# worldlife123/cbench_BaSIC

Hardware: AMD Instinct MI355X
Metric: encode+decode Mpix/s (higher is better)
Workload: dtype f32; 1 GPU; hyperprior codec N=128 M=192 (lossy_graph_scalable_exp_hp), synthetic 3x256x256 images (image i = manual_seed(i), rand), 256 images per GPU per step resident in HBM, compress+decompress incl. bitstream D2H/H2D, 6 concurrent stream workers per GPU (step k on worker k mod W: whole batches, W in flight); images_per_gpu=256, workers=6, rans_waves_per_workgroup=8, batches_in_flight=6, parallelism=image-sharded x1, RCCL all-reduce of metric sums

## Files before the change

cbench_basic_amd/_lib.py:

```python
import ctypes
import os

_HERE = os.path.dirname(os.path.abspath(__file__))
LIB_PATH = os.path.join(_HERE, "libbasic_hip.so")

OK, ERR_INVALID, ERR_NOT_INIT, ERR_HIP, ERR_OVERFLOW, ERR_NO_DEVICE = 0, -1, -2, -3, -4, -5
IMAGE_CHW, IMAGE_HWC = 0, 1
PIXEL_U8, PIXEL_F32 = 0, 1


class BasicHipError(RuntimeError):
    pass


class BasicHipInvalid(BasicHipError, ValueError):
    """A call the library refuses (BASIC_ERR_INVALID / BASIC_ERR_NOT_INIT): a ValueError, as the reference's pybind11 layer
    raises, and like every other failure of the library a BasicHipError."""


_lib = None

c_i32p = ctypes.c_void_p
_I, _L, _P, _F = ctypes.c_int, ctypes.c_int64, ctypes.c_void_p, ctypes.c_float

# ... 41 lines not shown
    "basic_rate_refine_dev": (_I, [_P, _I, _I, _P, _I, _P, _P, _P]),
    "basic_hp_session_set_rate_targets": (_I, [_P, _P, _I, _P, _I, _I]),
    "basic_hp_session_rate_result": (_I, [_P, _P, _P, _P, _I]),
    "basic_eb_quantize_index_dev": (_I, [_P, _P, _I, _I, _I, _P, _P, _P, _P]),
    "basic_eb_dequantize_dev": (_I, [_P, _P, _I, _I, _I, _P, _P]),
    "basic_i32_to_f32_dev": (_I, [_P, _L, _P, _P]),
    "basic_pgm_gauss_encode_group_dev": (_I, [_P, _P, _I, _I, _I, _P, _L, _P, _I, _P, _P, _L, _L, _P, _P]),
    "basic_pgm_gauss_index_group_dev": (_I, [_P, _I, _I, _I, _P, _L, _P, _I, _P, _L, _L, _P]),
    "basic_pgm_gauss_scatter_group_dev": (_I, [_P, _P, _I, _I, _I, _P, _L, _L, _L, _P, _P]),
    "basic_gauss_nll_per_image_dev": (_I, [_P, _P, _I, _I, _I, _I, _F, _F, _P, _P]),
    "basic_gauss_nll_per_image_q_dev": (_I, [_P, _P, _I, _I, _I, _P, _I, _F, _F, _P, _P]),
    "basic_eb_nll_per_image_dev": (_I, [_P, _P, _I, _I, _I, _F, _P, _P]),
    "basic_conv_plan_create": (_I, [_P, _P, _I, _I, _I, _I, _I, _I, _I, _I, _P, _P, _I, _I, _P]),
    "basic_conv_plan_out_hw": (_I, [_P, _I, _I, _P, _P]),
    "basic_conv_forward_dev": (_I, [_P, _P, _I, _I, _I, _P, _P]),
    "basic_conv_plan_channels": (_I, [_P, _P, _P]),
    "basic_hp_session_create": (_I, [_P, _I, _P, _I, _P, _I, _P, _I, _P, _I, _P, _P, _I, _F, _P, _P]),
    "basic_hp_encode_bound": (_L, [_P, _I, _I, _I]),
    "basic_hp_encode_images": (_I, [_P, _P, _I, _I, _I, _I, _P, _L, _P, _P]),
    "basic_hp_encode_result": (_I, [_P, _P, _L, _P]),
    "basic_hp_decoded_shape": (_I, [_P, _P, _L, _P, _P, _P, _P]),
    "basic_hp_decode_images": (_I, [_P, _P, _L, _P, _L, _P]),
    "basic_image_u8_to_f32_dev": (_I, [_P, _I, _I, _I, _I, _I, _P, _P]),
    "basic_image_f32_to_u8_dev": (_I, [_P, _I, _I, _I, _I, _I, _P, _P]),
    "basic_image_sse_u8_dev": (_I, [_P, _I, _P, _I, _I, _I, _I, _I, _P, _P]),
    "basic_image_tiles_u8_to_f32_dev": (_I, [_P, _I, _I, _I, _I, _I, _I, _I, _I, _I, _I, _I, _I, _P, _P]),
    "basic_image_tiles_f32_to_u8_dev": (_I, [_P, _I, _I, _I, _I, _I, _I, _I, _I, _I, _I, _I, _P, _I, _I, _I, _P]),
    "basic_image_tiles_overlap_u8_to_f32_dev": (_I, [_P, _I, _I, _I, _I, _I, _I, _I, _I, _I, _I, _I, _I, _P, _P]),
    "basic_image_tiles_blend_dev": (_I, [_P, _I, _I, _I, _I, _I, _I, _I, _I, _I, _I, _I, _P, _I, _I, _P]),
    "basic_image_tiles_last_path": (_I, [_P]),
# ... 102 lines not shown
```

cbench_basic_amd/csrc/conv.hip:

```cpp
#include "common.h"

#include <algorithm>
#include <cmath>
#include <cstdlib>
#include <cstring>
#include <new>
#include <vector>

using namespace basic;

namespace {
thread_local bool g_dynamic_tiles = false;
}
namespace basic {
bool set_dynamic_tiles(bool on)
{
    const bool prev = g_dynamic_tiles;
    g_dynamic_tiles = on;
    return prev;
}
}

namespace {

// ... 15 lines not shown
constexpr int kPSlotsFused = 6;
constexpr int kFusedCK = 4;
constexpr int kMaxCoutPerLaunch = 192;
constexpr int kSplitBelowBlocks = 384;
constexpr int kPackTail = 32 * 32 * 8 + 2048;

struct TapLaunch {
    const float *in;
    float *out;
    const float *wpack;
    const float *wrow;
    const float *bias;
    int64_t split_wstride;
    const float *gammaT;
    const float *beta;
    int batch, cin, cin_pad, cout, coutp;
    int out_ctotal, co_base;
    int in_h, in_w, out_h, out_w;
    int mh, mw;
    int s_in, s_out, oy0, ox0;
    int ntaps, dymin, dxmin;
    int tb_log, th_log, tw_log;
    int ph, pw, pwp;
    int patch4;
    int act;
    int tiles_y, tiles_x;
    signed char dy[kMaxTaps], dx[kMaxTaps];
};

__device__ __forceinline__ int xcd_tile(int b, int n)
// ... 655 lines not shown
        }
    };
    if (gdn) {
        __syncthreads();
        const f32x4 *src = reinterpret_cast<const f32x4 *>(g.gammaT);
        f32x4 *dst = reinterpret_cast<f32x4 *>(gl);
#pragma unroll
        for (int sl = 0; sl < 128 * 32 * 4 / 4 / kSplitThreads; ++sl) dst[sl * kSplitThreads + tid_e] = src[sl * kSplitThreads + tid_e];
        __syncthreads();
    }
    finish(acc);
    finish(acc2);

    const Pos ep = pos_of(tid_e);
    const int my = ep.my, mx = ep.mx, be = b0 + ep.tb;
    if (my < g.mh && mx < g.mw && be < g.batch) {
        const int oy = my * g.s_out + g.oy0, ox = mx * g.s_out + g.ox0;
        const int64_t oplane = static_cast<int64_t>(g.out_h) * g.out_w;
        float *o = g.out + (static_cast<int64_t>(be) * g.out_ctotal + g.co_base) * oplane + static_cast<int64_t>(oy) * g.out_w + ox;
#pragma unroll
        for (int m = 0; m < MT; ++m)
#pragma unroll
            for (int r = 0; r < 16; ++r) {
                const int co = 32 * m + 8 * (r >> 2) + 4 * khalf_e + (r & 3);
                if (co < g.cout) {
                    f32x2 v2;
                    v2[0] = apply_act(acc[m][r], g.act);
                    v2[1] = apply_act(acc2[m][r], g.act);
                    *reinterpret_cast<f32x2 *>(o + co * oplane) = v2;
                }
            }
    }
}

template <int KH, bool PATCH>
hipError_t launch_split(const TapLaunch &g, const u32x4 *ws, const int *kw, const unsigned *amax, int blocks, hipStream_t st)
{
    const hipError_t e = ensure_max_lds(reinterpret_cast<const void *>(conv_split_f16_kernel<KH, 3, 2, PATCH>));
    if (e != hipSuccess) return e;
    hipLaunchKernelGGL((conv_split_f16_kernel<KH, 3, 2, PATCH>), dim3(blocks), dim3(kSplitThreads),
                       PATCH ? kSplitLdsPatchBytes : kSplitLdsBytes, st, g, ws, kw, amax);
    return hipGetLastError();
}

constexpr int kFirstSlots = 10;

// ... 975 lines not shown
    BASIC_HIP_TRY(hipGetLastError());
    return BASIC_OK;
}
}

extern "C" int basic_conv_plan_launches(const basic_conv_plan *p, int batch, int in_h, int in_w)
{
    int oh = 0, ow = 0;
    if (!p || batch < 1 || basic_conv_plan_out_hw(p, in_h, in_w, &oh, &ow)) return -1;
    if (p->d_wsm) return 1;
    int n = 0;
    for_each_launch(p, choose_launches(p, batch, oh, ow, nullptr), oh, ow, [&](const Chunk &, const Phase &, int, int) { ++n; return BASIC_OK; });
    return n;
}

extern "C" int basic_conv_forward_dev(const basic_conv_plan *p, const float *d_in, int batch, int in_h, int in_w,
                                      float *d_out, void *hip_stream)
{
    BASIC_REQUIRE(p && d_in && d_out && batch >= 1, "conv_forward: bad argument");
    int oh = 0, ow = 0;
    int rc = basic_conv_plan_out_hw(p, in_h, in_w, &oh, &ow);
    if (rc) return rc;
    if (p->d_wsm) return launch_small_deconv(p, d_in, batch, in_h, in_w, d_out, as_stream(hip_stream));
    const LaunchChoice choice = choose_launches(p, batch, oh, ow, d_out);
    bool amax_done = false;
    return for_each_launch(p, choice, oh, ow, [&](const Chunk &ch, const Phase &ph, int mh, int mw) -> int {
        TapLaunch g{};
        g.in = d_in; g.out = d_out; g.wpack = ph.d_wpack; g.wrow = ph.d_wrow; g.split_wstride = ph.split_wstride; g.bias = ch.d_bias; g.gammaT = p->d_gammaT; g.beta = p->d_beta;
        g.batch = batch; g.cin = p->cin; g.cin_pad = ph.ntaps ? ph.cin_pad : 0; g.cout = ch.cout; g.coutp = ch.coutp; g.out_ctotal = p->cout; g.co_base = ch.co0;
        g.in_h = in_h; g.in_w = in_w; g.out_h = oh; g.out_w = ow;
        g.s_in = p->s_in; g.s_out = p->s_out; g.oy0 = ph.oy0; g.ox0 = ph.ox0;
        g.mh = mh; g.mw = mw;
        g.ntaps = ph.ntaps; g.dymin = ph.dymin; g.dxmin = ph.dxmin;
        std::memcpy(g.dy, ph.dy, sizeof(g.dy));
        std::memcpy(g.dx, ph.dx, sizeof(g.dx));
        g.act = p->act;
        const int kCK = ph.ck;
        if (choice.split_f16 && ph.d_wsplit) {
            const TileShape ts = tile_shape(g.mh, g.mw, kSplitWaves * 32);
            const int tw = ts.tw, th = ts.th, tb = ts.tb;
            if (static_cast<int64_t>(tb) * p->cin * in_h * in_w * 4 < (1ll << 31)) {
// ... 1 lines not shown
                g.tiles_y = (g.mh + th - 1) / th;
                g.tiles_x = (g.mw + tw - 1) / tw;
                const int blocks = ((batch + tb - 1) / tb) * g.tiles_y * g.tiles_x;
                hipStream_t st = as_stream(hip_stream);
                const u32x4 *ws = static_cast<const u32x4 *>(ph.d_wsplit);
                BASIC_REQUIRE(ph.kw == 3 && ph.kwb == 2 && (ph.kh == 3 || ph.kh == 2), "conv_forward: split-fp16 plan / kernel instantiation mismatch");
                if (!amax_done) {
                    auto *pm = const_cast<basic_conv_plan *>(p);
                    if (pm->amax_cap < batch) {
                        if (pm->d_amax) BASIC_HIP_TRY(hipFree(pm->d_amax));
                        pm->d_amax = nullptr; pm->amax_cap = 0;
                        BASIC_HIP_TRY(hipMalloc(&pm->d_amax, sizeof(unsigned) * batch));
                        pm->amax_cap = batch;
                    }
                    BASIC_HIP_TRY(hipMemsetAsync(pm->d_amax, 0, sizeof(unsigned) * batch, st));
                    const int64_t n = static_cast<int64_t>(p->cin) * in_h * in_w;
                    const int per_img = static_cast<int>(std::min<int64_t>(64, std::max<int64_t>(1, n / 4096)));
                    hipLaunchKernelGGL(image_absmax_kernel, dim3(batch * per_img), dim3(256), 0, st, d_in, n, per_img, pm->d_amax);
                    BASIC_HIP_TRY(hipGetLastError());
                    amax_done = true;
                }
                const bool patch = choice.split_patch && g.s_in == 1 && tb * (th + ph.kh - 1) * (tw + ph.kw - 1) <= kSplitPatchPos;
                const unsigned *am = p->d_amax;
                const hipError_t e = ph.kh == 3 ? (patch ? launch_split<3, true>(g, ws, ph.d_wsplit_k, am, blocks, st) : launch_split<3, false>(g, ws, ph.d_wsplit_k, am, blocks, st))
                                                : (patch ? launch_split<2, true>(g, ws, ph.d_wsplit_k, am, blocks, st) : launch_split<2, false>(g, ws, ph.d_wsplit_k, am, blocks, st));
                BASIC_HIP_TRY(e);
                return BASIC_OK;
            }
        }
        const int threads = 64 * ph.waves, tile_pos = 32 * ph.waves;
        const TileShape ts = tile_shape(g.mh, g.mw, tile_pos);
        const int tw = ts.tw;
        int th = ts.th, tb = ts.tb;
        const bool first_layer_path = ch.mt == 4 && ch.nsplit == 1 && ph.waves == 8 && ph.kh == 5 && ph.kw == 5 &&
                                      ph.cin_pad == kCK && kCK == 4 && ch.cout == 128 && p->d_gammaT;
        g.ph = (th - 1) * g.s_in + ph.span_y;
        g.pw = (tw - 1) * g.s_in + ph.span_x;
        g.patch4 = (ph.waves == 8 && !first_layer_path && in_w % 4 == 0 && (reinterpret_cast<uintptr_t>(d_in) & 15) == 0) ? 1 : 0;
        g.pwp = g.patch4 ? (g.pw + 3 + 3) / 4 * 4 : (g.pw | 1);
        int punit = g.patch4 ? 4 : 1;
        const int mtp = mtile_pitch(ch.mt);
        const int wl_floats = g.ntaps * kCK * 32 * mtp, gam_floats = 32 * 32 * mtp;
        const int wl_pad = ((wl_floats > gam_floats ? wl_floats : gam_floats) + 4 * threads - 1) / (4 * threads) * (4 * threads);
        auto patch_slots_needed = [&](int tbv) { return (tbv * kCK * g.ph * g.pwp / punit + threads - 1) / threads; };
// ... 55 lines not shown
                default: set_error("conv_forward: fused phases need <= 4 accumulator tiles"); rc = BASIC_ERR_INVALID;
            }
            return rc;
        }
        switch (ch.mt) {
            case 1: rc = launch_mt<1>(g, ph.kh, ph.kw, ph.ck, ph.waves, blocks, ch.nsplit, lds_bytes, st); break;
            case 2: rc = launch_mt<2>(g, ph.kh, ph.kw, ph.ck, ph.waves, blocks, ch.nsplit, lds_bytes, st); break;
            case 3: rc = launch_mt<3>(g, ph.kh, ph.kw, ph.ck, ph.waves, blocks, ch.nsplit, lds_bytes, st); break;
            case 4: rc = launch_mt<4>(g, ph.kh, ph.kw, ph.ck, ph.waves, blocks, ch.nsplit, lds_bytes, st); break;
            case 5: rc = launch_mt<5>(g, ph.kh, ph.kw, ph.ck, ph.waves, blocks, ch.nsplit, lds_bytes, st); break;
            case 6: rc = launch_mt<6>(g, ph.kh, ph.kw, ph.ck, ph.waves, blocks, ch.nsplit, lds_bytes, st); break;
            default: set_error("conv_forward: cout > 192 unsupported"); rc = BASIC_ERR_INVALID;
        }
        return rc;
    });
}
```

cbench_basic_amd/csrc/entropy.hip:

```cpp
#include "ans_common.h"

using namespace basic;

namespace {

constexpr int kBlock = 256;

inline int grid_for(int64_t n)
{
    int64_t g = (n + kBlock - 1) / kBlock;
    if (g > 256 * 8) g = 256 * 8;
    if (g < 1) g = 1;
    return static_cast<int>(g);
}

__device__ __forceinline__ float round_even(float v) { return rintf(v); }

__global__ void gc_quantize_index_kernel(const float *__restrict__ y, const float *__restrict__ scales, int64_t n,
                                         const float *__restrict__ table, int table_len, float bound,
                                         int32_t *__restrict__ symbols, int32_t *__restrict__ indexes,
                                         float *__restrict__ yhat)
{
    extern __shared__ float s_table[];
    __shared__ int s_unsorted;
// ... 248 lines not shown
__global__ void eb_dequantize_kernel(const int32_t *__restrict__ symbols, const float *__restrict__ medians,
                                     int64_t total, int channels, int hw, float *__restrict__ zhat)
{
    for (int64_t i = static_cast<int64_t>(blockIdx.x) * blockDim.x + threadIdx.x; i < total;
         i += static_cast<int64_t>(gridDim.x) * blockDim.x) {
        const int c = static_cast<int>((i / hw) % channels);
        zhat[i] = static_cast<float>(symbols[i]) + medians[c];
    }
}

__global__ void i32_to_f32_kernel(const int32_t *__restrict__ in, int64_t n, float *__restrict__ out)
{
    for (int64_t i = static_cast<int64_t>(blockIdx.x) * blockDim.x + threadIdx.x; i < n;
         i += static_cast<int64_t>(gridDim.x) * blockDim.x)
        out[i] = static_cast<float>(in[i]);
}

__global__ void lanes_pack_kernel(const int32_t *__restrict__ sym, const int32_t *__restrict__ idx, int64_t total, int positions,
                                  int lanes, int width, int32_t *__restrict__ sym_out, int32_t *__restrict__ idx_out)
{
    for (int64_t i = static_cast<int64_t>(blockIdx.x) * blockDim.x + threadIdx.x; i < total;
         i += static_cast<int64_t>(gridDim.x) * blockDim.x) {
        const int64_t run = i / width;
        const int l = static_cast<int>(i - run * width);
        const int64_t bk = run / positions;
        const int p = static_cast<int>(run - bk * positions);
        const int64_t b = bk / lanes;
        const int k = static_cast<int>(bk - b * lanes);
        const int64_t src = ((b * positions + p) * lanes + k) * width + l;
        sym_out[i] = sym[src];
// ... 338 lines not shown
    hipLaunchKernelGGL(eb_dequantize_kernel, dim3(grid_for(total)), dim3(kBlock), 0, as_stream(hip_stream), d_symbols,
                       d_medians, total, channels, hw, d_zhat);
    BASIC_HIP_TRY(hipGetLastError());
    return BASIC_OK;
}

extern "C" int basic_i32_to_f32_dev(const int32_t *d_in, int64_t n, float *d_out, void *hip_stream)
{
    BASIC_REQUIRE(d_in && d_out && n >= 0, "i32_to_f32: bad argument");
    if (n == 0) return BASIC_OK;
    hipLaunchKernelGGL(i32_to_f32_kernel, dim3(grid_for(n)), dim3(kBlock), 0, as_stream(hip_stream), d_in, n, d_out);
    BASIC_HIP_TRY(hipGetLastError());
    return BASIC_OK;
}

extern "C" int basic_lanes_pack_dev(const int32_t *d_sym, const int32_t *d_idx, int batch, int positions, int channels, int lanes,
                                    int32_t *d_sym_out, int32_t *d_idx_out, void *hip_stream)
{
    BASIC_REQUIRE(d_sym && d_idx && d_sym_out && d_idx_out && batch >= 1 && positions >= 1 && channels >= 1 && lanes >= 1 &&
                      channels % lanes == 0 && d_sym_out != d_sym && d_idx_out != d_idx,
                  "lanes_pack: bad argument");
    const int64_t total = static_cast<int64_t>(batch) * positions * channels;
    hipLaunchKernelGGL(lanes_pack_kernel, dim3(grid_for(total)), dim3(kBlock), 0, as_stream(hip_stream), d_sym, d_idx, total, positions,
                       lanes, channels / lanes, d_sym_out, d_idx_out);
    BASIC_HIP_TRY(hipGetLastError());
    return BASIC_OK;
}

extern "C" int basic_group_lanes_pack_dev(const int32_t *d_sym, const int32_t *d_idx, int batch, int64_t n, const int64_t *d_bases,
                                          int groups, int lanes, int32_t *d_sym_out, int32_t *d_idx_out, void *hip_stream)
// ... 108 lines not shown
```

cbench_basic_amd/csrc/session.hip:

```cpp
#include "common.h"

#include <cstring>
#include <map>
#include <mutex>
#include <vector>

using namespace basic;

constexpr int kMaxTokenLanes = 4;


namespace {

struct DBuf {
    void *p = nullptr;
    size_t cap = 0;
    int ensure(size_t bytes)
    {
        if (bytes <= cap) return BASIC_OK;
        if (p) (void)hipFree(p);
        p = nullptr;
        cap = 0;
        const size_t want = bytes + bytes / 4 + 256;
        BASIC_HIP_TRY(hipMalloc(&p, want));
// ... 78 lines not shown
    int rans_waves = 0;
    int lanes = 1;
    int res_lanes = 1;
    std::vector<float> qsteps;
    HBuf h_steps;
    DBuf d_steps;
    hipEvent_t steps_done = nullptr;
    std::vector<int64_t> rate_budget;
    std::vector<float> rate_cand;
    int rate_passes = 0, rate_res_batch = 0;
    HBuf h_rate, h_rate_out;
    DBuf d_rate_in, d_rate_bits, d_rate_cand[2], d_rate_out;
    hipEvent_t rate_up = nullptr;
    DBuf d_medians, d_table;
    DBuf act[2], d_x, d_y, d_z, d_zhat, d_prior, d_scales;
    DBuf z_sym, z_idx, y_sym, y_idx, seg_z, seg_y, slots_z, slots_y, nw, off, packed, words, woff, state, pos;
    HBuf h_nw, h_words, h_in;
    std::vector<int64_t> off_z, off_y;
    int res_batch = 0, res_zh = 0, res_zw = 0, res_yh = 0, res_yw = 0;
    hipEvent_t in_done = nullptr;
    hipStream_t side = nullptr;
    hipEvent_t fork = nullptr, join = nullptr;
    bool use_token = false;
    int token_lanes = 0;
    hipEvent_t enc_phase = nullptr, dec_phase = nullptr;
    hipStream_t copy = nullptr;
    hipEvent_t x_free = nullptr, x_ready = nullptr;
    bool x_read_pending = false;
    DBuf u8_in, u8_out, d_xhat;
    hipEvent_t u8_free = nullptr, xhat_free = nullptr;
    bool u8_read_pending = false, xhat_read_pending = false;
    ~basic_hp_session();
};

namespace {

int run_chain(basic_hp_session *s, const std::vector<const basic_conv_plan *> &plans, const float *d_in, int batch, int h, int w,
              DBuf *out_buf, float *d_final, int *oh_out, int *ow_out, hipStream_t st)
{
    const float *cur = d_in;
    int flip = 0;
    for (size_t i = 0; i < plans.size(); ++i) {
        int oh = 0, ow = 0, co = 0;
        int rc = basic_conv_plan_out_hw(plans[i], h, w, &oh, &ow);
        if (rc) return rc;
        rc = basic_conv_plan_channels(plans[i], nullptr, &co);
        if (rc) return rc;
        const size_t bytes = sizeof(float) * static_cast<size_t>(batch) * co * oh * ow;
        float *dst;
        if (i + 1 == plans.size()) {
            if (d_final) dst = d_final;
            else { rc = out_buf->ensure(bytes); if (rc) return rc; dst = out_buf->as<float>(); }
        } else {
            rc = s->act[flip].ensure(bytes);
            if (rc) return rc;
            dst = s->act[flip].as<float>();
            flip ^= 1;
        }
        rc = basic_conv_forward_dev(plans[i], cur, batch, h, w, dst, st);
        if (rc) return rc;
        cur = dst;
        h = oh;
        w = ow;
    }
    if (oh_out) *oh_out = h;
    if (ow_out) *ow_out = w;
    return BASIC_OK;
}

int chain_out_hw(const std::vector<const basic_conv_plan *> &plans, int h, int w, int *oh, int *ow)
{
    for (const auto *p : plans) {
        int a = 0, b = 0;
        int rc = basic_conv_plan_out_hw(p, h, w, &a, &b);
// ... 680 lines not shown
    if (rc) return rc;
    const int n_steps = static_cast<int>(s->qsteps.size());
    if (!n_steps) {
        rc = basic_gc_quantize_index_dev(d_scales, d_scales, batch * ny, s->d_table.as<float>(), s->n_scales, s->scale_bound,
                                         s->y_sym.as<int32_t>(), s->y_idx.as<int32_t>(), nullptr, st);
    } else {
        rc = upload_qsteps(s, st);
        if (!rc)
            rc = basic_gc_quantize_index_q_dev(d_scales, d_scales, batch * ny, ny, s->d_steps.as<float>(), n_steps, s->d_table.as<float>(),
                                               s->n_scales, s->scale_bound, s->y_sym.as<int32_t>(), s->y_idx.as<int32_t>(), nullptr, st);
    }
    if (rc) return rc;
    rc = basic_rans_decode_batch_dev(s->y_tables, d_wy, d_oy, s->y_idx.as<int32_t>(), s->seg_y.as<int64_t>(), sy, s->y_sym.as<int32_t>(),
                                     s->state.as<uint64_t>() + batch, s->pos.as<int64_t>() + batch, st);
    if (rc) return rc;
    if (!n_steps) rc = basic_i32_to_f32_dev(s->y_sym.as<int32_t>(), batch * ny, s->d_y.as<float>(), st);
    else rc = basic_gc_dequantize_q_dev(s->y_sym.as<int32_t>(), batch * ny, ny, s->d_steps.as<float>(), n_steps, s->d_y.as<float>(), st);
    if (rc) return rc;
    rc = rejoin(s, caller_st, st);
    if (rc) return rc;
    st = caller_st;
    TokenPhase phase(s, st, &s->dec_phase);
    if (phase.rc) return phase.rc;
    rc = run_chain(s, s->g_s, s->d_y.as<float>(), batch, yh, yw, nullptr, d_xhat, nullptr, nullptr, st);
    const int rc2 = phase.close();
    return rc ? rc : rc2;
}

}

extern "C" int basic_hp_decode_images(basic_hp_session *s, const uint8_t *data, int64_t len, float *d_xhat,
                                      int64_t xhat_capacity_floats, void *hip_stream)
{
    BASIC_REQUIRE(s && d_xhat, "hp_decode_images: bad argument");
    return decode_body(s, data, len, d_xhat, xhat_capacity_floats, as_stream(hip_stream));
}

extern "C" int basic_hp_decode_images_u8(basic_hp_session *s, const uint8_t *data, int64_t len, int layout, uint8_t *xhat,
                                         int xhat_on_host, int64_t xhat_capacity_bytes, void *hip_stream)
// ... 29 lines not shown
```

cbench_basic_amd/nn/kernels.py:

```python
import contextlib
import ctypes
import os

import numpy as np
import torch

from .. import _lib

ACT_NONE, ACT_RELU, ACT_LEAKY_RELU, ACT_GDN, ACT_IGDN = 0, 1, 2, 3, 4


def _dev(t, dtype=None):
    if not isinstance(t, torch.Tensor) or not t.is_cuda:
        raise _lib.BasicHipError("cbench_basic_amd kernels need tensors on the MI355X (got a CPU tensor); "
                                 "there is no CPU fallback")
    if dtype is not None and t.dtype != dtype:
        raise TypeError(f"expected {dtype}, got {t.dtype}")
    return t.contiguous()


def _stream():
    return torch.cuda.current_stream().cuda_stream


# ... 31 lines not shown
                _lib.lib().basic_conv_plan_destroy(h)
            except Exception:
                pass

    def out_hw(self, h, w):
        oh, ow = ctypes.c_int(), ctypes.c_int()
        _lib.check(_lib.lib().basic_conv_plan_out_hw(self._h, int(h), int(w), ctypes.byref(oh), ctypes.byref(ow)))
        return oh.value, ow.value

    def flops(self, batch, h, w):
        return int(_lib.lib().basic_conv_plan_flops(self._h, int(batch), int(h), int(w)))

    def launches(self, batch, h, w):
        return int(_lib.lib().basic_conv_plan_launches(self._h, int(batch), int(h), int(w)))

    def __call__(self, x, out=None):
        x = _dev(x, torch.float32)
        B, C, H, W = x.shape
        if C != self.cin:
            raise ValueError(f"conv plan expects {self.cin} input channels, got {C}")
        oh, ow = self.out_hw(H, W)
        if out is None:
            out = torch.empty((B, self.cout, oh, ow), device=x.device, dtype=torch.float32)
        _lib.check(_lib.lib().basic_conv_forward_dev(self._h, x.data_ptr(), B, H, W, out.data_ptr(), _stream()))
        return out


MCONV_KERNEL_NONE, MCONV_KERNEL_GATHER, MCONV_KERNEL_BLOCK, MCONV_KERNEL_DMA = -1, 0, 1, 2


def mconv_choose(cin, cout, ksize, in_groups, out_groups, batch, h, w, n_pos):
    k = ctypes.c_int(MCONV_KERNEL_NONE)
    _lib.check(_lib.lib().basic_mconv_choose(int(cin), int(cout), int(ksize), int(in_groups), int(out_groups), int(batch), int(h),
                                             int(w), int(n_pos), ctypes.byref(k)))
    return k.value


class MaskedConvPlan:

# ... 395 lines not shown

def eb_dequantize(sym, medians):
    sym, medians = _dev(sym, torch.int32), _dev(medians, torch.float32)
    B, C = sym.shape[0], sym.shape[1]
    hw = sym.numel() // (B * C)
    zhat = torch.empty(sym.shape, device=sym.device, dtype=torch.float32)
    _lib.check(_lib.lib().basic_eb_dequantize_dev(sym.data_ptr(), medians.data_ptr(), B, C, hw, zhat.data_ptr(), _stream()))
    return zhat


def i32_to_f32(sym):
    sym = _dev(sym, torch.int32)
    out = torch.empty(sym.shape, device=sym.device, dtype=torch.float32)
    _lib.check(_lib.lib().basic_i32_to_f32_dev(sym.data_ptr(), sym.numel(), out.data_ptr(), _stream()))
    return out


def mse_per_image(a, b):
    a, b = _dev(a, torch.float32), _dev(b, torch.float32)
    out = torch.empty((a.shape[0],), device=a.device, dtype=torch.float32)
    _lib.check(_lib.lib().basic_mse_per_image_dev(a.data_ptr(), b.data_ptr(), a.shape[0], a.numel() // a.shape[0], out.data_ptr(), _stream()))
    return out


def ms_ssim_per_image(x, y, data_range=1.0, return_terms=False, workspace=None):
    if not (isinstance(x, torch.Tensor) and isinstance(y, torch.Tensor)) or x.dim() != 4 or x.shape != y.shape:
        raise ValueError("ms_ssim_per_image takes two [B, C, H, W] tensors of one shape")
    x, y = _dev(x).float().contiguous(), _dev(y).float().contiguous()
    if y.device != x.device:
        raise ValueError("ms_ssim_per_image: the two batches live on different devices")
# ... 589 lines not shown
```

cbench_basic_amd/nn/models/google.py:

```python
import torch
import torch.nn as nn

from ..layers.gdn import GDN
from .. import kernels as K


def conv(in_channels, out_channels, kernel_size=5, stride=2):
    return nn.Conv2d(in_channels, out_channels, kernel_size=kernel_size, stride=stride, padding=kernel_size // 2)


def deconv(in_channels, out_channels, kernel_size=5, stride=2):
    return nn.ConvTranspose2d(in_channels, out_channels, kernel_size=kernel_size, stride=stride,
                              output_padding=stride - 1, padding=kernel_size // 2)


def compile_sequential(seq, cin_active=None, cout_actives=None):
    layers = list(seq)
    plans, i = [], 0
    while i < len(layers):
        m = layers[i]
        if not isinstance(m, (nn.Conv2d, nn.ConvTranspose2d)):
            raise TypeError(f"transform must start a fused group with a convolution, got {type(m).__name__}")
        act, gamma, beta = K.ACT_NONE, None, None
        if i + 1 < len(layers):
# ... 31 lines not shown

    def plans(self):
        key = self._key()
        if self._plans is None or key != self._plan_key:
            self._plans = compile_sequential(self.model)
            self._plan_key = key
        return self._plans

    def flops(self, batch, h, w):
        total = 0
        for p in self.plans():
            total += p.flops(batch, h, w)
            h, w = p.out_hw(h, w)
        return total

    def _forward(self, x):
        for p in self.plans():
            x = p(x)
        return x

    def forward(self, input, in_channel_gains=None, out_channel_gains=None, **kwargs):
        if in_channel_gains is not None:
            input = input * in_channel_gains.reshape(1, -1, 1, 1)
        output = self._forward(input)
        if out_channel_gains is not None:
            output = output * out_channel_gains.reshape(1, -1, 1, 1)
        return output


class HyperpriorAnalysisModel(BasicHyperpriorModule):
    def __init__(self, N, M, in_channels=3, **kwargs):
        super().__init__()
        self.in_channels, self.N, self.M = in_channels, N, M
# ... 44 lines not shown
```

include/basic_hip.h:

```cpp
#ifndef BASIC_HIP_H
#define BASIC_HIP_H

#include <stdint.h>

#ifdef __cplusplus
extern "C" {
#endif

#define BASIC_OK 0
#define BASIC_ERR_INVALID (-1)
#define BASIC_ERR_NOT_INIT (-2)
#define BASIC_ERR_HIP (-3)
#define BASIC_ERR_OVERFLOW (-4)
#define BASIC_ERR_NO_DEVICE (-5)

const char *basic_last_error(void);
int basic_device_count(int *count);
int basic_set_device(int ordinal);
int basic_stream_synchronize(void *hip_stream);

typedef struct basic_rans_tables basic_rans_tables;

int basic_pmf_to_quantized_cdf(const float *pmf, int n, int precision, int32_t *cdf_out );

// ... 89 lines not shown
#define BASIC_RATE_NO_FIT 0x40000000
int basic_rate_select_dev(const uint64_t *d_bits, int n_images, int segs_per_image, int64_t per_seg, const float *d_cand, int n_cand,
                          int cand_per_image, const int32_t *d_extra_words, const int64_t *d_budget, float *d_steps_out,
                          int32_t *d_choice, int64_t *d_pred_bytes, void *hip_stream);
int basic_rate_refine_dev(const float *d_cand_in, int cand_per_image, int n_cand, const int32_t *d_choice, int n_images,
                          const float *d_t, float *d_cand_out, void *hip_stream);
int basic_lanes_pack_dev(const int32_t *d_sym, const int32_t *d_idx, int batch, int positions, int channels, int lanes,
                         int32_t *d_sym_out, int32_t *d_idx_out, void *hip_stream);
int basic_group_lanes_pack_dev(const int32_t *d_sym, const int32_t *d_idx, int batch, int64_t n, const int64_t *d_bases, int groups,
                               int lanes, int32_t *d_sym_out, int32_t *d_idx_out, void *hip_stream);
int basic_eb_quantize_index_dev(const float *d_z, const float *d_medians, int batch, int channels, int hw,
                                int32_t *d_symbols, int32_t *d_indexes, float *d_zhat, void *hip_stream);
int basic_eb_dequantize_dev(const int32_t *d_symbols, const float *d_medians, int batch, int channels,
                            int hw, float *d_zhat, void *hip_stream);
int basic_i32_to_f32_dev(const int32_t *d_in, int64_t n, float *d_out, void *hip_stream);

int basic_pgm_gauss_encode_group_dev(const float *d_y, const float *d_params, int batch, int channels, int hw,
                                     const int32_t *d_elems, int64_t n_elems, const float *d_table,
                                     int table_len, int32_t *d_symbols, int32_t *d_indexes, int64_t per_image,
                                     int64_t out_base, float *d_ybuf, void *hip_stream);
int basic_pgm_gauss_index_group_dev(const float *d_params, int batch, int channels, int hw,
                                    const int32_t *d_elems, int64_t n_elems, const float *d_table,
                                    int table_len, int32_t *d_indexes, int64_t per_image, int64_t out_base,
                                    void *hip_stream);
int basic_pgm_gauss_scatter_group_dev(const int32_t *d_symbols, const float *d_params, int batch, int channels,
                                      int hw, const int32_t *d_elems, int64_t n_elems, int64_t per_image,
                                      int64_t in_base, float *d_ybuf, void *hip_stream);

int basic_gauss_nll_per_image_dev(const float *d_q, const float *d_scales_or_params, int batch, int channels, int hw,
                                  int interleaved_mean_scale, float scale_bound, float likelihood_bound, float *d_nll,
// ... 7 lines not shown

#define BASIC_ACT_NONE 0
#define BASIC_ACT_RELU 1
#define BASIC_ACT_LEAKY_RELU 2
#define BASIC_ACT_GDN 3
#define BASIC_ACT_IGDN 4

int basic_conv_plan_create(const float *weight, const float *bias, int cin, int cout, int ksize, int stride,
                           int padding, int output_padding, int transposed, int activation,
                           const float *gamma, const float *beta, int cin_active, int cout_active,
                           basic_conv_plan **out);
int basic_conv_plan_out_hw(const basic_conv_plan *p, int in_h, int in_w, int *out_h, int *out_w);
int basic_conv_plan_channels(const basic_conv_plan *p, int *cin_active, int *cout_active);
int basic_conv_forward_dev(const basic_conv_plan *p, const float *d_in, int batch, int in_h, int in_w,
                           float *d_out, void *hip_stream);
void basic_conv_plan_destroy(basic_conv_plan *p);
int64_t basic_conv_plan_flops(const basic_conv_plan *p, int batch, int in_h, int in_w);
int basic_conv_plan_launches(const basic_conv_plan *p, int batch, int in_h, int in_w);

typedef struct basic_mconv_plan basic_mconv_plan;
int basic_mconv_plan_create(const float *weight, const float *bias, int cin, int cout, int ksize,
                            int in_groups, int out_groups, int allow_same_topogroup, int activation,
                            basic_mconv_plan **out);
int basic_mconv_forward_pos_dev(const basic_mconv_plan *p, const float *d_x, const int32_t *d_topo_in,
                                const int32_t *d_topo_out, int batch, int h, int w, const int32_t *d_pos,
                                int64_t n_pos, float *d_y, int out_channels_total, int out_channel_offset,
                                void *hip_stream);
int basic_mconv_forward_step_dev(const basic_mconv_plan *p, const float *d_x, const int32_t *d_topo_in,
                                 const int32_t *d_topo_out, int batch, int h, int w, const int32_t *d_pos,
                                 int64_t n_pos, float *d_y, int out_channels_total, int out_channel_offset,
// ... 179 lines not shown
```

Before: 885.5 Mpix/s.

## Fuse per-image absmax into producer conv epilogue and int-to-float conversion in decoder

The split f16 conv path used to run a separate image_absmax pass over each layer's input before the conv. Now the layer that produces that input computes the per-image absmax in its epilogue with wave ballot reduction and atomicMax. In the decoder, the i32-to-f32 symbol conversion also produces the absmax. This removes a full extra read of every activation tensor and one launch per layer in the g_s chain. The cost is extra register work and atomics in the conv epilogue, plus a memset of the per-layer amax buffer.

```diff
diff --git a/cbench_basic_amd/_lib.py b/cbench_basic_amd/_lib.py
--- a/cbench_basic_amd/_lib.py
+++ b/cbench_basic_amd/_lib.py
@@ -79,6 +79,9 @@
     "basic_conv_plan_create": (_I, [_P, _P, _I, _I, _I, _I, _I, _I, _I, _I, _P, _P, _I, _I, _P]),
     "basic_conv_plan_out_hw": (_I, [_P, _I, _I, _P, _P]),
     "basic_conv_forward_dev": (_I, [_P, _P, _I, _I, _I, _P, _P]),
+    "basic_conv_forward_amax_dev": (_I, [_P, _P, _I, _I, _I, _P, _P, _P, _P]),
+    "basic_conv_plan_wants_amax": (_I, [_P]),
+    "basic_i32_to_f32_amax_dev": (_I, [_P, _L, _I, _P, _P, _P]),
     "basic_conv_plan_channels": (_I, [_P, _P, _P]),
     "basic_hp_session_create": (_I, [_P, _I, _P, _I, _P, _I, _P, _I, _P, _I, _P, _P, _I, _F, _P, _P]),
     "basic_hp_encode_bound": (_L, [_P, _I, _I, _I]),
diff --git a/cbench_basic_amd/csrc/conv.hip b/cbench_basic_amd/csrc/conv.hip
--- a/cbench_basic_amd/csrc/conv.hip
+++ b/cbench_basic_amd/csrc/conv.hip
@@ -53,6 +53,7 @@
     int64_t split_wstride;
     const float *gammaT;
     const float *beta;
+    unsigned *amax_out;
     int batch, cin, cin_pad, cout, coutp;
     int out_ctotal, co_base;
     int in_h, in_w, out_h, out_w;
@@ -738,6 +739,7 @@
 
     const Pos ep = pos_of(tid_e);
     const int my = ep.my, mx = ep.mx, be = b0 + ep.tb;
+    unsigned amx = 0;
     if (my < g.mh && mx < g.mw && be < g.batch) {
         const int oy = my * g.s_out + g.oy0, ox = mx * g.s_out + g.ox0;
         const int64_t oplane = static_cast<int64_t>(g.out_h) * g.out_w;
@@ -752,8 +754,23 @@
                     v2[0] = apply_act(acc[m][r], g.act);
                     v2[1] = apply_act(acc2[m][r], g.act);
                     *reinterpret_cast<f32x2 *>(o + co * oplane) = v2;
-                }
-            }
+                    amx = max(amx, max(__float_as_uint(v2[0]) & 0x7FFFFFFFu, __float_as_uint(v2[1]) & 0x7FFFFFFFu));
+                }
+            }
+    }
+
+    if (g.amax_out) {
+        unsigned long long todo = __ballot(amx != 0);
+        while (todo) {
+            const int leader = __builtin_ctzll(todo);
+            const int img = __shfl(be, leader);
+            const bool mine = be == img;
+            unsigned v = mine ? amx : 0u;
+#pragma unroll
+            for (int off = 32; off > 0; off >>= 1) v = max(v, static_cast<unsigned>(__shfl_xor(static_cast<int>(v), off)));
+            if (static_cast<int>(__lane_id()) == leader) atomicMax(g.amax_out + img, v);
+            todo &= ~__ballot(mine);
+        }
     }
 }
 
@@ -1759,17 +1776,52 @@
     return n;
 }
 
+namespace {
+int queue_image_absmax(const float *d_x, int batch, int64_t n, unsigned *amax, hipStream_t st)
+{
+    const int per_img = static_cast<int>(std::min<int64_t>(64, std::max<int64_t>(1, n / 4096)));
+    hipLaunchKernelGGL(image_absmax_kernel, dim3(batch * per_img), dim3(256), 0, st, d_x, n, per_img, amax);
+    BASIC_HIP_TRY(hipGetLastError());
+    return BASIC_OK;
+}
+}
+
+extern "C" int basic_conv_plan_wants_amax(const basic_conv_plan *p)
+{
+    if (!p) return 0;
+    const char *f32_env = getenv("BASIC_CONV_F32");
+    if (f32_env && atoi(f32_env) != 0) return 0;
+    for (const auto *list : {&p->chunks, &p->split})
+        for (const Chunk &ch : *list)
+            for (const auto *phs : {&ch.phases, &ch.fused})
+                for (const Phase &ph : *phs)
+                    if (ph.d_wsplit) return 1;
+    return 0;
+}
+
 extern "C" int basic_conv_forward_dev(const basic_conv_plan *p, const float *d_in, int batch, int in_h, int in_w,
                                       float *d_out, void *hip_stream)
+{
+    return basic_conv_forward_amax_dev(p, d_in, batch, in_h, in_w, d_out, nullptr, nullptr, hip_stream);
+}
+
+extern "C" int basic_conv_forward_amax_dev(const basic_conv_plan *p, const float *d_in, int batch, int in_h, int in_w,
+                                           float *d_out, const unsigned *d_amax_in, unsigned *d_amax_out, void *hip_stream)
 {
     BASIC_REQUIRE(p && d_in && d_out && batch >= 1, "conv_forward: bad argument");
     int oh = 0, ow = 0;
     int rc = basic_conv_plan_out_hw(p, in_h, in_w, &oh, &ow);
     if (rc) return rc;
-    if (p->d_wsm) return launch_small_deconv(p, d_in, batch, in_h, in_w, d_out, as_stream(hip_stream));
+    const int64_t out_per_image = static_cast<int64_t>(p->cout) * oh * ow;
+    if (p->d_wsm) {
+        rc = launch_small_deconv(p, d_in, batch, in_h, in_w, d_out, as_stream(hip_stream));
+        if (!rc && d_amax_out) rc = queue_image_absmax(d_out, batch, out_per_image, d_amax_out, as_stream(hip_stream));
+        return rc;
+    }
     const LaunchChoice choice = choose_launches(p, batch, oh, ow, d_out);
-    bool amax_done = false;
-    return for_each_launch(p, choice, oh, ow, [&](const Chunk &ch, const Phase &ph, int mh, int mw) -> int {
+    bool amax_done = d_amax_in != nullptr;
+    bool amax_out_missed = false;
+    rc = for_each_launch(p, choice, oh, ow, [&](const Chunk &ch, const Phase &ph, int mh, int mw) -> int {
         TapLaunch g{};
         g.in = d_in; g.out = d_out; g.wpack = ph.d_wpack; g.wrow = ph.d_wrow; g.split_wstride = ph.split_wstride; g.bias = ch.d_bias; g.gammaT = p->d_gammaT; g.beta = p->d_beta;
         g.batch = batch; g.cin = p->cin; g.cin_pad = ph.ntaps ? ph.cin_pad : 0; g.cout = ch.cout; g.coutp = ch.coutp; g.out_ctotal = p->cout; g.co_base = ch.co0;
@@ -1801,20 +1853,20 @@
                         pm->amax_cap = batch;
                     }
                     BASIC_HIP_TRY(hipMemsetAsync(pm->d_amax, 0, sizeof(unsigned) * batch, st));
-                    const int64_t n = static_cast<int64_t>(p->cin) * in_h * in_w;
-                    const int per_img = static_cast<int>(std::min<int64_t>(64, std::max<int64_t>(1, n / 4096)));
-                    hipLaunchKernelGGL(image_absmax_kernel, dim3(batch * per_img), dim3(256), 0, st, d_in, n, per_img, pm->d_amax);
-                    BASIC_HIP_TRY(hipGetLastError());
+                    const int rca = queue_image_absmax(d_in, batch, static_cast<int64_t>(p->cin) * in_h * in_w, pm->d_amax, st);
+                    if (rca) return rca;
                     amax_done = true;
                 }
                 const bool patch = choice.split_patch && g.s_in == 1 && tb * (th + ph.kh - 1) * (tw + ph.kw - 1) <= kSplitPatchPos;
-                const unsigned *am = p->d_amax;
+                const unsigned *am = d_amax_in ? d_amax_in : p->d_amax;
+                g.amax_out = d_amax_out;
                 const hipError_t e = ph.kh == 3 ? (patch ? launch_split<3, true>(g, ws, ph.d_wsplit_k, am, blocks, st) : launch_split<3, false>(g, ws, ph.d_wsplit_k, am, blocks, st))
                                                 : (patch ? launch_split<2, true>(g, ws, ph.d_wsplit_k, am, blocks, st) : launch_split<2, false>(g, ws, ph.d_wsplit_k, am, blocks, st));
                 BASIC_HIP_TRY(e);
                 return BASIC_OK;
             }
         }
+        amax_out_missed = true;
         const int threads = 64 * ph.waves, tile_pos = 32 * ph.waves;
         const TileShape ts = tile_shape(g.mh, g.mw, tile_pos);
         const int tw = ts.tw;
@@ -1900,4 +1952,6 @@
         }
         return rc;
     });
-}
+    if (!rc && d_amax_out && amax_out_missed) rc = queue_image_absmax(d_out, batch, out_per_image, d_amax_out, as_stream(hip_stream));
+    return rc;
+}
diff --git a/cbench_basic_amd/csrc/entropy.hip b/cbench_basic_amd/csrc/entropy.hip
--- a/cbench_basic_amd/csrc/entropy.hip
+++ b/cbench_basic_amd/csrc/entropy.hip
@@ -286,6 +286,47 @@
     for (int64_t i = static_cast<int64_t>(blockIdx.x) * blockDim.x + threadIdx.x; i < n;
          i += static_cast<int64_t>(gridDim.x) * blockDim.x)
         out[i] = static_cast<float>(in[i]);
+}
+
+__global__ __launch_bounds__(kBlock) void i32_to_f32_amax_kernel(const int32_t *__restrict__ in, int64_t n, int per_img,
+                                                                 float *__restrict__ out, unsigned *__restrict__ amax)
+{
+    typedef int i32x4 __attribute__((ext_vector_type(4)));
+    typedef float f32x4 __attribute__((ext_vector_type(4)));
+    __shared__ unsigned wave_max[kBlock / 64];
+    const int img = blockIdx.x / per_img, part = blockIdx.x - img * per_img;
+    const int32_t *src = in + img * n;
+    float *dst = out + img * n;
+    unsigned m = 0;
+    if (((reinterpret_cast<uintptr_t>(src) | reinterpret_cast<uintptr_t>(dst) | static_cast<uintptr_t>(n * 4)) & 15) == 0) {
+        const i32x4 *s4 = reinterpret_cast<const i32x4 *>(src);
+        f32x4 *d4 = reinterpret_cast<f32x4 *>(dst);
+        for (int64_t i = part * kBlock + threadIdx.x; i < n / 4; i += per_img * kBlock) {
+            const i32x4 s = s4[i];
+            f32x4 v;
+#pragma unroll
+            for (int e = 0; e < 4; ++e) {
+                v[e] = static_cast<float>(s[e]);
+                m = max(m, __float_as_uint(v[e]) & 0x7FFFFFFFu);
+            }
+            d4[i] = v;
+        }
+    } else {
+        for (int64_t i = part * kBlock + threadIdx.x; i < n; i += per_img * kBlock) {
+            const float v = static_cast<float>(src[i]);
+            dst[i] = v;
+            m = max(m, __float_as_uint(v) & 0x7FFFFFFFu);
+        }
+    }
+#pragma unroll
+    for (int off = 32; off > 0; off >>= 1) m = max(m, static_cast<unsigned>(__shfl_xor(static_cast<int>(m), off)));
+    if ((threadIdx.x & 63) == 0) wave_max[threadIdx.x >> 6] = m;
+    __syncthreads();
+    if (threadIdx.x == 0) {
+#pragma unroll
+        for (int w = 1; w < kBlock / 64; ++w) m = max(m, wave_max[w]);
+        if (m) atomicMax(amax + img, m);
+    }
 }
 
 __global__ void lanes_pack_kernel(const int32_t *__restrict__ sym, const int32_t *__restrict__ idx, int64_t total, int positions,
@@ -654,6 +695,19 @@
     return BASIC_OK;
 }
 
+extern "C" int basic_i32_to_f32_amax_dev(const int32_t *d_in, int64_t n_per_image, int batch, float *d_out, unsigned *d_amax,
+                                         void *hip_stream)
+{
+    BASIC_REQUIRE(d_in && d_out && d_amax && n_per_image >= 0 && batch >= 0, "i32_to_f32_amax: bad argument");
+    if (n_per_image == 0 || batch == 0) return BASIC_OK;
+    const int per_img = static_cast<int>(std::min<int64_t>(64, std::max<int64_t>(1, n_per_image / (16 * kBlock))));
+    BASIC_REQUIRE(static_cast<int64_t>(batch) * per_img < (1ll << 31), "i32_to_f32_amax: batch too large");
+    hipLaunchKernelGGL(i32_to_f32_amax_kernel, dim3(batch * per_img), dim3(kBlock), 0, as_stream(hip_stream), d_in, n_per_image, per_img,
+                       d_out, d_amax);
+    BASIC_HIP_TRY(hipGetLastError());
+    return BASIC_OK;
+}
+
 extern "C" int basic_lanes_pack_dev(const int32_t *d_sym, const int32_t *d_idx, int batch, int positions, int channels, int lanes,
                                     int32_t *d_sym_out, int32_t *d_idx_out, void *hip_stream)
 {
diff --git a/cbench_basic_amd/csrc/session.hip b/cbench_basic_amd/csrc/session.hip
--- a/cbench_basic_amd/csrc/session.hip
+++ b/cbench_basic_amd/csrc/session.hip
@@ -116,6 +116,7 @@
     hipEvent_t rate_up = nullptr;
     DBuf d_medians, d_table;
     DBuf act[2], d_x, d_y, d_z, d_zhat, d_prior, d_scales;
+    DBuf d_amax;
     DBuf z_sym, z_idx, y_sym, y_idx, seg_z, seg_y, slots_z, slots_y, nw, off, packed, words, woff, state, pos;
     HBuf h_nw, h_words, h_in;
     std::vector<int64_t> off_z, off_y;
@@ -137,8 +138,19 @@
 
 namespace {
 
+int zero_chain_amax(basic_hp_session *s, size_t layers, int batch, hipStream_t st, unsigned **out)
+{
+    const size_t bytes = sizeof(unsigned) * layers * static_cast<size_t>(batch);
+    const int rc = s->d_amax.ensure(bytes);
+    if (rc) return rc;
+    BASIC_HIP_TRY(hipMemsetAsync(s->d_amax.as<unsigned>(), 0, bytes, st));
+    *out = s->d_amax.as<unsigned>();
+    return BASIC_OK;
+}
+
 int run_chain(basic_hp_session *s, const std::vector<const basic_conv_plan *> &plans, const float *d_in, int batch, int h, int w,
-              DBuf *out_buf, float *d_final, int *oh_out, int *ow_out, hipStream_t st)
+              DBuf *out_buf, float *d_final, int *oh_out, int *ow_out, hipStream_t st, unsigned *d_amax = nullptr,
+              bool first_amax = false)
 {
     const float *cur = d_in;
     int flip = 0;
@@ -159,7 +171,13 @@
             dst = s->act[flip].as<float>();
             flip ^= 1;
         }
-        rc = basic_conv_forward_dev(plans[i], cur, batch, h, w, dst, st);
+        const unsigned *am_in = nullptr;
+        unsigned *am_out = nullptr;
+        if (d_amax) {
+            if ((i > 0 || first_amax) && basic_conv_plan_wants_amax(plans[i])) am_in = d_amax + i * static_cast<size_t>(batch);
+            if (i + 1 < plans.size() && basic_conv_plan_wants_amax(plans[i + 1])) am_out = d_amax + (i + 1) * static_cast<size_t>(batch);
+        }
+        rc = basic_conv_forward_amax_dev(plans[i], cur, batch, h, w, dst, am_in, am_out, st);
         if (rc) return rc;
         cur = dst;
         h = oh;
@@ -870,7 +888,12 @@
     rc = basic_rans_decode_batch_dev(s->y_tables, d_wy, d_oy, s->y_idx.as<int32_t>(), s->seg_y.as<int64_t>(), sy, s->y_sym.as<int32_t>(),
                                      s->state.as<uint64_t>() + batch, s->pos.as<int64_t>() + batch, st);
     if (rc) return rc;
-    if (!n_steps) rc = basic_i32_to_f32_dev(s->y_sym.as<int32_t>(), batch * ny, s->d_y.as<float>(), st);
+    unsigned *d_amax = nullptr;
+    rc = zero_chain_amax(s, s->g_s.size(), batch, st, &d_amax);
+    if (rc) return rc;
+    const bool first_amax = !n_steps && !s->g_s.empty() && basic_conv_plan_wants_amax(s->g_s[0]);
+    if (first_amax) rc = basic_i32_to_f32_amax_dev(s->y_sym.as<int32_t>(), ny, batch, s->d_y.as<float>(), d_amax, st);
+    else if (!n_steps) rc = basic_i32_to_f32_dev(s->y_sym.as<int32_t>(), batch * ny, s->d_y.as<float>(), st);
     else rc = basic_gc_dequantize_q_dev(s->y_sym.as<int32_t>(), batch * ny, ny, s->d_steps.as<float>(), n_steps, s->d_y.as<float>(), st);
     if (rc) return rc;
     rc = rejoin(s, caller_st, st);
@@ -878,7 +901,7 @@
     st = caller_st;
     TokenPhase phase(s, st, &s->dec_phase);
     if (phase.rc) return phase.rc;
-    rc = run_chain(s, s->g_s, s->d_y.as<float>(), batch, yh, yw, nullptr, d_xhat, nullptr, nullptr, st);
+    rc = run_chain(s, s->g_s, s->d_y.as<float>(), batch, yh, yw, nullptr, d_xhat, nullptr, nullptr, st, d_amax, first_amax);
     const int rc2 = phase.close();
     return rc ? rc : rc2;
 }
diff --git a/cbench_basic_amd/nn/kernels.py b/cbench_basic_amd/nn/kernels.py
--- a/cbench_basic_amd/nn/kernels.py
+++ b/cbench_basic_amd/nn/kernels.py
@@ -69,7 +69,10 @@
     def launches(self, batch, h, w):
         return int(_lib.lib().basic_conv_plan_launches(self._h, int(batch), int(h), int(w)))
 
-    def __call__(self, x, out=None):
+    def wants_amax(self):
+        return bool(_lib.lib().basic_conv_plan_wants_amax(self._h))
+
+    def __call__(self, x, out=None, amax_in=None, amax_out=None):
         x = _dev(x, torch.float32)
         B, C, H, W = x.shape
         if C != self.cin:
@@ -77,7 +80,15 @@
         oh, ow = self.out_hw(H, W)
         if out is None:
             out = torch.empty((B, self.cout, oh, ow), device=x.device, dtype=torch.float32)
-        _lib.check(_lib.lib().basic_conv_forward_dev(self._h, x.data_ptr(), B, H, W, out.data_ptr(), _stream()))
+        for a in (amax_in, amax_out):
+            if a is not None and (not a.is_cuda or a.dtype != torch.int32 or a.numel() != B or not a.is_contiguous()):
+                raise ValueError("per-image maxima are contiguous int32 [batch] device tensors")
+        if amax_in is None and amax_out is None:
+            _lib.check(_lib.lib().basic_conv_forward_dev(self._h, x.data_ptr(), B, H, W, out.data_ptr(), _stream()))
+        else:
+            _lib.check(_lib.lib().basic_conv_forward_amax_dev(
+                self._h, x.data_ptr(), B, H, W, out.data_ptr(), amax_in.data_ptr() if amax_in is not None else None,
+                amax_out.data_ptr() if amax_out is not None else None, _stream()))
         return out
 
 
@@ -503,6 +514,16 @@
     out = torch.empty(sym.shape, device=sym.device, dtype=torch.float32)
     _lib.check(_lib.lib().basic_i32_to_f32_dev(sym.data_ptr(), sym.numel(), out.data_ptr(), _stream()))
     return out
+
+
+def i32_to_f32_amax(sym):
+    sym = _dev(sym, torch.int32)
+    B = sym.shape[0]
+    out = torch.empty(sym.shape, device=sym.device, dtype=torch.float32)
+    amax = torch.zeros((B,), device=sym.device, dtype=torch.int32)
+    _lib.check(_lib.lib().basic_i32_to_f32_amax_dev(sym.data_ptr(), sym.numel() // B if B else 0, B, out.data_ptr(), amax.data_ptr(),
+                                                    _stream()))
+    return out, amax
 
 
 def mse_per_image(a, b):
diff --git a/cbench_basic_amd/nn/models/google.py b/cbench_basic_amd/nn/models/google.py
--- a/cbench_basic_amd/nn/models/google.py
+++ b/cbench_basic_amd/nn/models/google.py
@@ -69,9 +69,14 @@
             h, w = p.out_hw(h, w)
         return total
 
-    def _forward(self, x):
-        for p in self.plans():
-            x = p(x)
+    def _forward(self, x, amax_in=None):
+        plans = self.plans()
+        wants = [p.wants_amax() for p in plans]
+        amax = torch.zeros((len(plans), x.shape[0]), device=x.device, dtype=torch.int32) if any(wants[1:]) else None
+        for i, p in enumerate(plans):
+            a_in = (amax_in if i == 0 else amax[i]) if wants[i] else None
+            a_out = amax[i + 1] if i + 1 < len(plans) and wants[i + 1] else None
+            x = p(x, amax_in=a_in, amax_out=a_out)
         return x
 
     def forward(self, input, in_channel_gains=None, out_channel_gains=None, **kwargs):
diff --git a/include/basic_hip.h b/include/basic_hip.h
--- a/include/basic_hip.h
+++ b/include/basic_hip.h
@@ -127,6 +127,7 @@
 int basic_eb_dequantize_dev(const int32_t *d_symbols, const float *d_medians, int batch, int channels,
                             int hw, float *d_zhat, void *hip_stream);
 int basic_i32_to_f32_dev(const int32_t *d_in, int64_t n, float *d_out, void *hip_stream);
+int basic_i32_to_f32_amax_dev(const int32_t *d_in, int64_t n_per_image, int batch, float *d_out, unsigned *d_amax, void *hip_stream);
 
 int basic_pgm_gauss_encode_group_dev(const float *d_y, const float *d_params, int batch, int channels, int hw,
                                      const int32_t *d_elems, int64_t n_elems, const float *d_table,
@@ -164,6 +165,9 @@
 int basic_conv_plan_channels(const basic_conv_plan *p, int *cin_active, int *cout_active);
 int basic_conv_forward_dev(const basic_conv_plan *p, const float *d_in, int batch, int in_h, int in_w,
                            float *d_out, void *hip_stream);
+int basic_conv_forward_amax_dev(const basic_conv_plan *p, const float *d_in, int batch, int in_h, int in_w, float *d_out,
+                                const unsigned *d_amax_in, unsigned *d_amax_out, void *hip_stream);
+int basic_conv_plan_wants_amax(const basic_conv_plan *p);
 void basic_conv_plan_destroy(basic_conv_plan *p);
 int64_t basic_conv_plan_flops(const basic_conv_plan *p, int batch, int in_h, int in_w);
 int basic_conv_plan_launches(const basic_conv_plan *p, int batch, int in_h, int in_w);
```

Result: no change. 885.0 Mpix/s (-0.1%).
